# ningyu1991/InclusiveGAN

Hardware: AMD Instinct MI355X
Metric: training img/sec (whole node), CelebA 128x128 StyleGAN2+IMLE (higher is better)
Workload: dtype f32-equivalent (3x3 convs: 2-piece fp16 split, operands to <= 1 ulp of fp32, scales per pixel / per channel: no per-tensor window; fp32 sums)

## Files before the change

inclusivegan_amd/csrc/upfirdn2d.hip:

```cpp
#include "igan_common.h"
#include <hip/hip_fp16.h>
#include <cstdlib>

namespace {

struct FirTaps {
    float k[64];
};

struct UpfirdnArgs {
    const float* x;
    float* y;
    int upx, upy, downx, downy;
    int padx0, pady0;
    int majorDim, inH, inW, minorDim;
    int kernelH, kernelW;
    int outH, outW;
    int xcd_remap;
    const float* noise;
    const float* strength;
    const float* bias;
    int noise_bcast, act;
    float act_alpha, act_gain;
};

__host__ __device__ __forceinline__ int floor_div(int a, int b) {
    int c = a / b;
    if (c * b > a) c--;
    return c;
}

__device__ __forceinline__ float io_load(const float* p) { return *p; }
__device__ __forceinline__ float io_load(const __half* p) { return __half2float(*p); }
__device__ __forceinline__ void io_store(float* p, float v) { *p = v; }
__device__ __forceinline__ void io_store(__half* p, float v) { *p = __float2half(v); }

struct TapWalk { int j0, i0, n; };

__device__ __forceinline__ TapWalk tap_walk(int o, int down, int up, int pad0, int taps, int in) {
    const int u0 = o * down - pad0;
    const int j0 = (u0 >= 0) ? (up - u0 % up) % up : -u0;
    const int i0 = (u0 + j0) / up;
    const int by_taps = (j0 < taps) ? (taps - j0 + up - 1) / up : 0;
    const int by_samples = (i0 < in) ? in - i0 : 0;
    return TapWalk{j0, i0, min(by_taps, by_samples)};
}

template <typename T>
__global__ __launch_bounds__(256) void upfirdn2d_generic_kernel(UpfirdnArgs a, FirTaps taps) {
    const T* xin = reinterpret_cast<const T*>(a.x);
    T* yout = reinterpret_cast<T*>(a.y);
    const long long total = (long long)a.majorDim * a.outH * a.outW * a.minorDim;
    for (long long idx = (long long)blockIdx.x * blockDim.x + threadIdx.x; idx < total;
         idx += (long long)gridDim.x * blockDim.x) {
        long long t = idx;
        const int c = (int)(t % a.minorDim); t /= a.minorDim;
        const int ox = (int)(t % a.outW);    t /= a.outW;
        const int oy = (int)(t % a.outH);    t /= a.outH;
        const int m = (int)t;
        const TapWalk wy = tap_walk(oy, a.downy, a.upy, a.pady0, a.kernelH, a.inH);
        const TapWalk wx = tap_walk(ox, a.downx, a.upx, a.padx0, a.kernelW, a.inW);
        float v = 0.0f;
        for (int sy = 0; sy < wy.n; sy++) {
            const T* xrow = xin + (((long long)m * a.inH + wy.i0 + sy) * a.inW + wx.i0) * a.minorDim + c;
            const float* krow = taps.k + (wy.j0 + sy * a.upy) * a.kernelW + wx.j0;
            for (int sx = 0; sx < wx.n; sx++)
                v += io_load(xrow + (long long)sx * a.minorDim) * krow[sx * a.upx];
        }
        io_store(yout + idx, v);
    }
}

template <int TY, int TX, bool EPI = false>
__global__ __launch_bounds__(256) void upfirdn2d_fir4_kernel(UpfirdnArgs a, FirTaps taps) {
    const int cvecs = a.minorDim >> 2;
    const int strips = (a.outH + TY - 1) / TY;
    const int xgroups = (a.outW + TX - 1) / TX;
    const long long total = (long long)a.majorDim * strips * xgroups * cvecs;
    int bid = blockIdx.x;
    if (a.xcd_remap) {
        const int n = gridDim.x, q = n >> 3, r = n & 7, x = bid & 7;
        bid = (x < r ? x * (q + 1) : r * (q + 1) + (x - r) * q) + (bid >> 3);
    }
    const long long idx = (long long)bid * blockDim.x + threadIdx.x;
    if (idx >= total) return;
    long long t = idx;
    const int cv = (int)(t % cvecs); t /= cvecs;
    const int ox0 = (int)(t % xgroups) * TX; t /= xgroups;
    const int strip = (int)(t % strips); t /= strips;
    const int m = (int)t;
    const int oy0 = strip * TY;

    float4 acc[TY][TX];
#pragma unroll
    for (int i = 0; i < TY; i++)
#pragma unroll
        for (int j = 0; j < TX; j++) acc[i][j] = make_float4(0.f, 0.f, 0.f, 0.f);

    const int ix0 = ox0 - a.padx0;
    const float4* xbase = reinterpret_cast<const float4*>(a.x) + (long long)m * a.inH * a.inW * cvecs + cv;

#pragma unroll
    for (int r = 0; r < TY + 3; r++) {
        const int iy = oy0 + r - a.pady0;
        float4 v[TX + 3];
        const bool rowok = (iy >= 0) & (iy < a.inH);
#pragma unroll
        for (int c = 0; c < TX + 3; c++) {
            const int ix = ix0 + c;
            const bool ok = rowok & (ix >= 0) & (ix < a.inW);
            v[c] = ok ? xbase[((long long)iy * a.inW + ix) * cvecs] : make_float4(0.f, 0.f, 0.f, 0.f);
        }
#pragma unroll
        for (int ky = 0; ky < 4; ky++) {
            const int o = r - ky;
            if (o >= 0 && o < TY) {
#pragma unroll
                for (int j = 0; j < TX; j++)
#pragma unroll
                    for (int kx = 0; kx < 4; kx++) {
                        const float kv = taps.k[ky * 4 + kx];
                        acc[o][j].x += v[j + kx].x * kv;
                        acc[o][j].y += v[j + kx].y * kv;
                        acc[o][j].z += v[j + kx].z * kv;
                        acc[o][j].w += v[j + kx].w * kv;
                    }
            }
        }
    }

    float4* ybase = reinterpret_cast<float4*>(a.y) + (long long)m * a.outH * a.outW * cvecs + cv;
    float4 bb = make_float4(0.f, 0.f, 0.f, 0.f);
    float st = 0.f;
    if constexpr (EPI) {
        if (a.bias) bb = *reinterpret_cast<const float4*>(a.bias + 4 * cv);
        if (a.noise) st = a.strength[0];
    }
#pragma unroll
    for (int i = 0; i < TY; i++) {
        const int oy = oy0 + i;
#pragma unroll
        for (int j = 0; j < TX; j++)
            if (oy < a.outH && ox0 + j < a.outW) {
                float4 v = acc[i][j];
                if constexpr (EPI) {
                    const float nz = a.noise ? a.noise[((long long)(a.noise_bcast ? 0 : m) * a.outH + oy) * a.outW + ox0 + j] * st : 0.f;
                    const float e[4] = {v.x + nz + bb.x, v.y + nz + bb.y, v.z + nz + bb.z, v.w + nz + bb.w};
                    float o[4];
#pragma unroll
                    for (int q = 0; q < 4; q++) {
                        float t = e[q];
                        if (a.act == 2) t = t > 0.f ? t : 0.f;
                        if (a.act == 3) t = t > 0.f ? t : t * a.act_alpha;
                        o[q] = t * a.act_gain;
                    }
                    v = make_float4(o[0], o[1], o[2], o[3]);
                }
                ybase[((long long)oy * a.outW + ox0 + j) * cvecs] = v;
            }
    }
}

}

namespace {
struct FirEpilogue { const float* noise; const float* strength; const float* bias; int noise_bcast, act; float alpha, gain; };
int upfirdn_launch(hipStream_t stream, const igan_upfirdn2d_params* p, const FirEpilogue* epi, bool half_io = false);
}

extern "C" int igan_upfirdn2d(igan_stream_t stream_, const igan_upfirdn2d_params* p) {
    return upfirdn_launch((hipStream_t)stream_, p, nullptr);
}

extern "C" int igan_upfirdn2d_f16(igan_stream_t stream_, const igan_upfirdn2d_params* p) {
    return upfirdn_launch((hipStream_t)stream_, p, nullptr, true);
}

extern "C" int igan_upfirdn2d_ban(igan_stream_t stream_, const igan_upfirdn2d_params* p, const float* noise, const float* strength,
                                  int noise_bcast, const float* bias, int act, float alpha, float gain) {
    using namespace igan;
    IGAN_REQUIRE(act >= 1 && act <= 3, "upfirdn2d_ban: act must be 1 (linear), 2 (relu) or 3 (lrelu)");
    IGAN_REQUIRE(gain > 0.0f, "upfirdn2d_ban: gain must be positive");
    IGAN_REQUIRE((noise == nullptr) == (strength == nullptr), "upfirdn2d_ban: noise and strength go together");
    IGAN_REQUIRE(((uintptr_t)bias & 15) == 0, "upfirdn2d_ban: bias must be 16-byte aligned");
    FirEpilogue e{noise, strength, bias, noise_bcast, act, alpha, gain};
    return upfirdn_launch((hipStream_t)stream_, p, &e);
}

namespace {
int upfirdn_launch(hipStream_t stream, const igan_upfirdn2d_params* p, const FirEpilogue* epi, bool half_io) {
    using namespace igan;
    IGAN_REQUIRE(p != nullptr, "upfirdn2d: null params");
    IGAN_REQUIRE(p->x && p->k && p->y, "upfirdn2d: null buffer");
    IGAN_REQUIRE(p->upx >= 1 && p->upy >= 1, "upx and upy must be at least 1x1");
    IGAN_REQUIRE(p->downx >= 1 && p->downy >= 1, "downx and downy must be at least 1x1");
    IGAN_REQUIRE(p->kernelW >= 1 && p->kernelH >= 1, "kernel must be at least 1x1");
    IGAN_REQUIRE(p->kernelW * p->kernelH <= 64, "kernel too large (max 64 taps)");
    IGAN_REQUIRE(p->majorDim >= 1 && p->inH >= 1 && p->inW >= 1 && p->minorDim >= 1, "input must have rank 4 with positive dims");
    const int outW = (p->inW * p->upx + p->padx0 + p->padx1 - p->kernelW + p->downx) / p->downx;
    const int outH = (p->inH * p->upy + p->pady0 + p->pady1 - p->kernelH + p->downy) / p->downy;
    IGAN_REQUIRE(outW >= 1 && outH >= 1, "output must be at least 1x1");
    IGAN_REQUIRE(outW == p->outW && outH == p->outH, "upfirdn2d: outH/outW (%d,%d) do not match derived (%d,%d)", p->outH, p->outW, outH, outW);
    const long long in_elems = (long long)p->majorDim * p->inH * p->inW * p->minorDim;
    const long long out_elems = (long long)p->majorDim * outH * outW * p->minorDim;
    IGAN_REQUIRE(in_elems <= INT32_MAX, "input too large");
    IGAN_REQUIRE(out_elems <= INT32_MAX, "output too large");

    UpfirdnArgs a;
    a.x = p->x; a.y = p->y;
    a.upx = p->upx; a.upy = p->upy; a.downx = p->downx; a.downy = p->downy;
    a.padx0 = p->padx0; a.pady0 = p->pady0;
    a.majorDim = p->majorDim; a.inH = p->inH; a.inW = p->inW; a.minorDim = p->minorDim;
    a.kernelH = p->kernelH; a.kernelW = p->kernelW;
    a.outH = outH; a.outW = outW;
    static const bool fir_xcd = !(getenv("IGAN_FIR_XCD") && atoi(getenv("IGAN_FIR_XCD")) == 0);
    a.xcd_remap = fir_xcd ? 1 : 0;
    a.noise = epi ? epi->noise : nullptr; a.strength = epi ? epi->strength : nullptr; a.bias = epi ? epi->bias : nullptr;
    a.noise_bcast = epi ? epi->noise_bcast : 0; a.act = epi ? epi->act : 0;
    a.act_alpha = epi ? epi->alpha : 0.f; a.act_gain = epi ? epi->gain : 1.f;

    const bool aligned = (((uintptr_t)p->x | (uintptr_t)p->y) & 15) == 0;
    const bool fast = !half_io && p->upx == 1 && p->upy == 1 && p->downx == 1 && p->downy == 1 &&
                      p->kernelH <= 4 && p->kernelW <= 4 && (p->minorDim % 4) == 0 && aligned;
    FirTaps taps;
    for (int i = 0; i < 64; i++) taps.k[i] = 0.0f;
    if (fast) {
        for (int ky = 0; ky < p->kernelH; ky++)
            for (int kx = 0; kx < p->kernelW; kx++)
                taps.k[ky * 4 + kx] = p->k[(p->kernelH - 1 - ky) * p->kernelW + (p->kernelW - 1 - kx)];
        const int cvecs = p->minorDim / 4;
        static const int tx = getenv("IGAN_FIR_TX") ? atoi(getenv("IGAN_FIR_TX")) : 2;
        if (outH >= 8 && outW >= 16 && tx >= 2) {
            const long long total = (long long)p->majorDim * ceil_div(outH, 8) * ceil_div(outW, 2) * cvecs;
            if (epi) hipLaunchKernelGGL((upfirdn2d_fir4_kernel<8, 2, true>), dim3((int)ceil_div_ll(total, 256)), dim3(256), 0, stream, a, taps);
            else hipLaunchKernelGGL((upfirdn2d_fir4_kernel<8, 2>), dim3((int)ceil_div_ll(total, 256)), dim3(256), 0, stream, a, taps);
        } else if (outH >= 8) {
            const long long total = (long long)p->majorDim * ceil_div(outH, 8) * outW * cvecs;
            if (epi) hipLaunchKernelGGL((upfirdn2d_fir4_kernel<8, 1, true>), dim3((int)ceil_div_ll(total, 256)), dim3(256), 0, stream, a, taps);
            else hipLaunchKernelGGL((upfirdn2d_fir4_kernel<8, 1>), dim3((int)ceil_div_ll(total, 256)), dim3(256), 0, stream, a, taps);
        } else {
            const long long total = (long long)p->majorDim * ceil_div(outH, 2) * outW * cvecs;
            if (epi) hipLaunchKernelGGL((upfirdn2d_fir4_kernel<2, 1, true>), dim3((int)ceil_div_ll(total, 256)), dim3(256), 0, stream, a, taps);
            else hipLaunchKernelGGL((upfirdn2d_fir4_kernel<2, 1>), dim3((int)ceil_div_ll(total, 256)), dim3(256), 0, stream, a, taps);
        }
    } else {
        if (epi) return fail(IGAN_ERR_UNSUPPORTED, "upfirdn2d_ban: the epilogue rides on the FIR fast path only (up = down = 1, taps <= 4x4, minorDim %% 4 == 0, 16-byte aligned)");
        for (int ky = 0; ky < p->kernelH; ky++)
            for (int kx = 0; kx < p->kernelW; kx++)
                taps.k[ky * p->kernelW + kx] = p->k[(p->kernelH - 1 - ky) * p->kernelW + (p->kernelW - 1 - kx)];
        const int grid = (int)std::min<long long>(ceil_div_ll(out_elems, 256), 256 * 32);
        if (half_io) {
            for (int i = 0; i < 64; i++) taps.k[i] = (float)(_Float16)taps.k[i];
            hipLaunchKernelGGL(upfirdn2d_generic_kernel<__half>, dim3(grid), dim3(256), 0, stream, a, taps);
        } else {
            hipLaunchKernelGGL(upfirdn2d_generic_kernel<float>, dim3(grid), dim3(256), 0, stream, a, taps);
        }
    }
    IGAN_LAUNCH_CHECK("upfirdn2d launch");
    return IGAN_OK;
}
}
```

inclusivegan_amd/dnnlib/tflib/ops/upfirdn_2d.py:

```python
import numpy as np
import torch

from .... import hip_ops

_IMPLS = ('hip', 'cuda')


def _check_impl(impl):
    if impl not in _IMPLS:
        raise ValueError("impl must be 'hip' (or the reference's 'cuda'; got %r); the CPU reference lives in oracle/ and is not a product path" % (impl,))


def upfirdn_2d(x, k, upx=1, upy=1, downx=1, downy=1, padx0=0, padx1=0, pady0=0, pady1=0, impl='hip'):
    _check_impl(impl)
    k = np.asarray(k, dtype=np.float32)
    if x.dim() != 4:
        raise ValueError('input must have rank 4')
    for v in (upx, upy, downx, downy, padx0, padx1, pady0, pady1):
        assert isinstance(v, (int, np.integer))
    return hip_ops.UpFirDn2dFn.apply(x, k, int(upx), int(upy), int(downx), int(downy), int(padx0), int(padx1), int(pady0), int(pady1))


def filter_2d(x, k, gain=1, data_format='NCHW', impl='hip'):
    k = _setup_kernel(k) * gain
    p = k.shape[0] - 1
    return _simple_upfirdn_2d(x, k, pad0=(p+1)//2, pad1=p//2, data_format=data_format, impl=impl)

def upsample_2d(x, k=None, factor=2, gain=1, data_format='NCHW', impl='hip'):
    assert isinstance(factor, int) and factor >= 1
    if k is None:
        k = [1] * factor
    k = _setup_kernel(k) * (gain * (factor ** 2))
    p = k.shape[0] - factor
    return _simple_upfirdn_2d(x, k, up=factor, pad0=(p+1)//2+factor-1, pad1=p//2, data_format=data_format, impl=impl)

def downsample_2d(x, k=None, factor=2, gain=1, data_format='NCHW', impl='hip'):
    assert isinstance(factor, int) and factor >= 1
    if k is None:
        k = [1] * factor
    k = _setup_kernel(k) * gain
    p = k.shape[0] - factor
    return _simple_upfirdn_2d(x, k, down=factor, pad0=(p+1)//2, pad1=p//2, data_format=data_format, impl=impl)


def _to_nchw(x, data_format):
    assert data_format in ['NCHW', 'NHWC']
    return x if data_format == 'NCHW' else x.permute(0, 3, 1, 2)

def _from_nchw(y, data_format):
    return y if data_format == 'NCHW' else y.permute(0, 2, 3, 1)

def upsample_conv_2d(x, w, k=None, factor=2, gain=1, data_format='NCHW', impl='hip'):
    _check_impl(impl)
    assert isinstance(factor, int) and factor >= 1
    assert w.dim() == 4
    convH, convW, inC, outC = [int(d) for d in w.shape]
    assert convW == convH
    if factor != 2:
        raise NotImplementedError('upsample_conv_2d: only factor=2 is built (the only one the configs use)')
    if k is None:
        k = [1] * factor
    k = _setup_kernel(k) * (gain * (factor ** 2))
    p = (k.shape[0] - factor) - (convW - 1)
    xn = _to_nchw(x, data_format)
    if xn.shape[1] != inC:
        raise NotImplementedError('upsample_conv_2d: grouped convolution is not offered on the hip path')
    H, W = int(xn.shape[2]), int(xn.shape[3])
    geom = hip_ops.ConvGeom(convH, convW, 1, factor, convH - 1, convW - 1)
    y = hip_ops.conv2d(xn, w, geom, ((H - 1) * factor + convH, (W - 1) * factor + convW))
    y = _simple_upfirdn_2d(y, k, pad0=(p+1)//2+factor-1, pad1=p//2+1, data_format='NCHW', impl=impl)
    return _from_nchw(y, data_format)

def conv_downsample_2d(x, w, k=None, factor=2, gain=1, data_format='NCHW', impl='hip'):
    _check_impl(impl)
    assert isinstance(factor, int) and factor >= 1
    convH, convW, inC, outC = [int(d) for d in w.shape]
    assert convW == convH
    if k is None:
        k = [1] * factor
    k = _setup_kernel(k) * gain
    p = (k.shape[0] - factor) + (convW - 1)
    xn = _to_nchw(x, data_format)
    xn = _simple_upfirdn_2d(xn, k, pad0=(p+1)//2, pad1=p//2, data_format='NCHW', impl=impl)
    H, W = int(xn.shape[2]), int(xn.shape[3])
    geom = hip_ops.ConvGeom(convH, convW, factor, 1, 0, 0)
    y = hip_ops.conv2d(xn, w, geom, ((H - convH) // factor + 1, (W - convW) // factor + 1))
    return _from_nchw(y, data_format)


def _setup_kernel(k):
    k = np.asarray(k, dtype=np.float32)
    if k.ndim == 1:
        k = np.outer(k, k)
    k /= np.sum(k)
    assert k.ndim == 2
    assert k.shape[0] == k.shape[1]
    return k

def _simple_upfirdn_2d(x, k, up=1, down=1, pad0=0, pad1=0, data_format='NCHW', impl='hip'):
    assert data_format in ['NCHW', 'NHWC']
    assert x.dim() == 4
    y = x
    if data_format == 'NCHW':
        y = hip_ops.nhwc(y).permute(0, 2, 3, 1)
    y = upfirdn_2d(y, k, upx=up, upy=up, downx=down, downy=down, padx0=pad0, padx1=pad1, pady0=pad0, pady1=pad1, impl=impl)
    if data_format == 'NCHW':
        y = y.permute(0, 3, 1, 2)
    return y
```

inclusivegan_amd/hip_ops.py:

```python
import ctypes
import os
from collections import namedtuple

import numpy as np
import torch

from . import _abi

CL = torch.channels_last


def _stream():
    return ctypes.c_void_p(torch.cuda.current_stream().cuda_stream)


def _ptr(t):
    return ctypes.c_void_p(t.data_ptr()) if t is not None else ctypes.c_void_p(0)


def _require_cuda_f32(*ts):
    for t in ts:
        if t is None:
            continue
        if not t.is_cuda:
            raise RuntimeError('inclusivegan_amd kernels need tensors on a ROCm device (got %s); there is no CPU path' % t.device)
        if t.dtype != torch.float32:
            raise TypeError('inclusivegan_amd kernels are fp32 (got %s)' % t.dtype)


def _require_cuda_io(*ts):
    kinds = {t.dtype for t in ts if t is not None}
    for t in ts:
        if t is not None and not t.is_cuda:
            raise RuntimeError('inclusivegan_amd kernels need tensors on a ROCm device (got %s); there is no CPU path' % t.device)
    if len(kinds) != 1 or next(iter(kinds)) not in (torch.float32, torch.float16):
        raise TypeError('upfirdn_2d / fused_bias_act take float32 or float16 tensors of one type (got %s)' % sorted(str(k) for k in kinds))
    return next(iter(kinds)) == torch.float16


def _is_meta(t):
    return t.device.type == 'meta'


def _needed(ctx, i):
    if not ctx.needs_input_grad[i]:
        return False
    try:
        mask = getattr(ctx, 'input_is_tensor', None)
        j = i if mask is None else sum(1 for m in mask[:i] if m)
        node = ctx.next_functions[j][0]
        return node is not None and torch._C._will_engine_execute_node(node)
    except Exception:
        return True


def _mark_inputs(ctx, *inputs):
    ctx.input_is_tensor = [isinstance(t, torch.Tensor) for t in inputs]


def nhwc(x):
    return x.contiguous(memory_format=CL)


def empty_nchw(n, c, h, w, like):
    return torch.empty((n, c, h, w), device=like.device, dtype=torch.float32, memory_format=CL)



def upfirdn2d_raw(x, k, upx, upy, downx, downy, padx0, padx1, pady0, pady1, epilogue=None):
    k = np.ascontiguousarray(k, dtype=np.float32)
    if k.ndim != 2:
        raise ValueError('kernel must have rank 2')
    if x.dim() != 4:
        raise ValueError('input must have rank 4')
    major, in_h, in_w, minor = x.shape
    kh, kw = k.shape
    out_w = (in_w * upx + padx0 + padx1 - kw + downx) // downx
    out_h = (in_h * upy + pady0 + pady1 - kh + downy) // downy
    if out_w < 1 or out_h < 1:
        raise ValueError('output must be at least 1x1')
    if _is_meta(x):
        return torch.empty((major, out_h, out_w, minor), device='meta')
    lib = _abi.get_plugin()
    half = _require_cuda_io(x)
    if half and epilogue is not None:
        raise TypeError('upfirdn2d: the fused layer epilogue is a float32 path')
    x = x.contiguous()
    y = torch.empty((major, out_h, out_w, minor), device=x.device, dtype=x.dtype)
    p = _abi.UpFirDn2DParams(
        x=x.data_ptr(), k=k.ctypes.data, y=y.data_ptr(),
        upx=upx, upy=upy, downx=downx, downy=downy,
        padx0=padx0, padx1=padx1, pady0=pady0, pady1=pady1,
        majorDim=major, inH=in_h, inW=in_w, minorDim=minor,
        kernelH=kh, kernelW=kw, outH=out_h, outW=out_w)
    if epilogue is not None:
        noise, strength, bias, act_idx, alpha, gain = epilogue
        _require_cuda_f32(noise, strength, bias)
        if noise is not None:
            noise = noise.contiguous()
            if noise.numel() not in (out_h * out_w, major * out_h * out_w):
                raise ValueError('upfirdn2d epilogue: noise must hold [majorDim or 1, outH, outW] values')
        bcast = 1 if (noise is not None and noise.numel() == out_h * out_w and major > 1) else 0
        _abi.check(lib.igan_upfirdn2d_ban(_stream(), ctypes.byref(p), _ptr(noise), _ptr(strength if noise is not None else None), bcast,
                                          _ptr(bias.contiguous() if bias is not None else None), int(act_idx), float(alpha), float(gain)))
        return y
    _abi.check((lib.igan_upfirdn2d_f16 if half else lib.igan_upfirdn2d)(_stream(), ctypes.byref(p)))
    return y


def fir_ban_fusable(x, k, act_idx):
    k = np.asarray(k)
    return (_FIR_BAN and _second_order_depth == 0 and not _is_meta(x) and x.is_cuda and x.dim() == 4 and x.shape[1] % 4 == 0
            and act_idx in (1, 2, 3) and k.ndim == 2 and k.shape[0] <= 4 and k.shape[1] <= 4)


_FIR_BAN = os.environ.get('IGAN_FIR_BAN', '1') != '0'


class FirBanFn(torch.autograd.Function):

    @staticmethod
    def forward(ctx, x, k, pad0, pad1, b, noise, strength, act_idx, alpha, gain):
        _mark_inputs(ctx, x, k, pad0, pad1, b, noise, strength, act_idx, alpha, gain)
        k = np.asarray(k, dtype=np.float32)
        xh = nhwc(x).permute(0, 2, 3, 1)
        y = upfirdn2d_raw(xh, k, 1, 1, 1, 1, pad0, pad1, pad0, pad1, epilogue=(noise, strength, b, act_idx, alpha, gain))
        in_h, in_w = xh.shape[1], xh.shape[2]
        out_h, out_w = y.shape[1], y.shape[2]
        kh, kw = k.shape
        ctx.gargs = (np.ascontiguousarray(k[::-1, ::-1]), 1, 1, 1, 1, kw - pad0 - 1, in_w - out_w + pad0, kh - pad0 - 1, in_h - out_h + pad0)
        y = y.permute(0, 3, 1, 2)
        ctx.save_for_backward(y, noise)
        ctx.cfg = (act_idx, alpha, gain)
        ctx.has_b = b is not None
        return y

    @staticmethod
    def backward(ctx, dy):
        if torch.is_grad_enabled():
            raise NotImplementedError('fused FIR + epilogue: second-order gradients go through UpFirDn2dFn + BiasActNoiseFn (hip_ops.second_order())')
        y, noise = ctx.saved_tensors
        act_idx, alpha, gain = ctx.cfg
        need_b = ctx.has_b and _needed(ctx, 4)
        need_s = noise is not None and _needed(ctx, 6)
        nz = noise.expand(_noise_view(y)).contiguous() if noise is not None else None
        dxp, db, ds = bias_act_noise_bwd_raw(dy, y, nz, act_idx, alpha, gain, need_b)
        dx = None
        if _needed(ctx, 0):
            dx = upfirdn2d_raw(nhwc(dxp).permute(0, 2, 3, 1), *ctx.gargs).permute(0, 3, 1, 2)
        return dx, None, None, None, (db if need_b else None), None, (ds if need_s else None), None, None, None


class UpFirDn2dFn(torch.autograd.Function):

    @staticmethod
    def forward(ctx, x, k, upx, upy, downx, downy, padx0, padx1, pady0, pady1):
        k = np.asarray(k, dtype=np.float32)
        in_h, in_w = x.shape[1], x.shape[2]
        y = upfirdn2d_raw(x, k, upx, upy, downx, downy, padx0, padx1, pady0, pady1)
        out_h, out_w = y.shape[1], y.shape[2]
        kh, kw = k.shape
        gpadx0 = kw - padx0 - 1
        gpady0 = kh - pady0 - 1
        gpadx1 = in_w * upx - out_w * downx + padx0 - upx + 1
        gpady1 = in_h * upy - out_h * downy + pady0 - upy + 1
        ctx.gargs = (np.ascontiguousarray(k[::-1, ::-1]), downx, downy, upx, upy, gpadx0, gpadx1, gpady0, gpady1)
        return y

    @staticmethod
    def backward(ctx, dy):
        dx = UpFirDn2dFn.apply(dy, *ctx.gargs)
        return (dx,) + (None,) * 9



def _bias_layout(x, axis):
    if x.dim() == 4 and axis == 1 and x.is_contiguous(memory_format=CL):
        return x, x.shape[1], 1
    xc = x.contiguous()
    step = 1
    for d in xc.shape[axis + 1:]:
        step *= int(d)
    return xc, int(xc.shape[axis]), step


def fused_bias_act_raw(x, b, ref, grad, act_idx, alpha, gain, size_b, step_b):
    if _is_meta(x):
        return torch.empty_like(x)
    lib = _abi.get_plugin()
    half = _require_cuda_io(x, b, ref)
    y = torch.empty_like(x)
    p = _abi.FusedBiasActParams(
        x=x.data_ptr(), b=(b.data_ptr() if b is not None else None),
        ref=(ref.data_ptr() if ref is not None else None), y=y.data_ptr(),
        grad=grad, act=act_idx, alpha=float(alpha), gain=float(gain),
        sizeX=x.numel(), sizeB=size_b, stepB=step_b)
    _abi.check((lib.igan_fused_bias_act_f16 if half else lib.igan_fused_bias_act)(_stream(), ctypes.byref(p)))
    return y


def bias_grad_raw(dx, size_b, step_b):
    lib = _abi.get_plugin()
    if dx.dtype == torch.float16:
        return dx.reshape(-1, size_b, step_b).float().sum(dim=(0, 2)).to(torch.float16)
    _require_cuda_f32(dx)
    n = dx.numel()
    ws_floats = lib.igan_bias_grad_workspace_floats(n, size_b, step_b)
    ws = torch.empty((max(int(ws_floats), 1),), device=dx.device, dtype=torch.float32)
    db = torch.empty((size_b,), device=dx.device, dtype=torch.float32)
    _abi.check(lib.igan_bias_grad(_stream(), _ptr(dx), _ptr(db), _ptr(ws), n, size_b, step_b))
    return db


def _match_layout(t, ref):
    if t.shape == ref.shape and t.stride() == ref.stride():
        return t
    out = torch.empty_like(ref)
    out.copy_(t)
    return out


class _FbaGradFn(torch.autograd.Function):

    @staticmethod
    def forward(ctx, dy, bias_term, ref, axis, act_idx, alpha, gain, size_b, step_b, zero_2nd, xrecv=None):
        ctx.cfg = (axis, act_idx, alpha, gain, size_b, step_b, zero_2nd)
        ctx.has_bias_term = bias_term is not None
        dyl = _match_layout(dy, ref)
        ctx.save_for_backward(ref, *(() if zero_2nd else (dyl, bias_term) if bias_term is not None else (dyl,)))
        return fused_bias_act_raw(dyl, bias_term, ref, 1, act_idx, alpha, gain, size_b, step_b)

    @staticmethod
    def backward(ctx, d_dx):
        ref = ctx.saved_tensors[0]
        axis, act_idx, alpha, gain, size_b, step_b, zero_2nd = ctx.cfg
        d_dy = _FbaGradFn.apply(d_dx, None, ref, axis, act_idx, alpha, gain, size_b, step_b, True) if zero_2nd else None
        d_x = None
        if not zero_2nd:
            with torch.no_grad():
                g = _match_layout(d_dx, ref)
                d_dy = fused_bias_act_raw(g, None, ref, 1, act_idx, alpha, gain, size_b, step_b)
                if ctx.needs_input_grad[10]:
                    dy = ctx.saved_tensors[1]
                    if ctx.has_bias_term:
                        view = [1] * dy.dim(); view[axis] = -1
                        dy = dy + ctx.saved_tensors[2].view(*view)
                    d_x = fused_bias_act_raw(g, None, ref, 2, act_idx, alpha, gain, size_b, step_b) * dy
        d_bias_term = None
        if ctx.has_bias_term:
            d_bias_term = _BiasGradFn.apply(d_dy, axis, size_b, step_b)
        return (d_dy, d_bias_term) + (None,) * 8 + (d_x,)


class _BiasGradFn(torch.autograd.Function):

    @staticmethod
    def forward(ctx, dx, axis, size_b, step_b):
        ctx.shape = dx.shape
        ctx.axis = axis
        return bias_grad_raw(dx, size_b, step_b)

    @staticmethod
    def backward(ctx, d_db):
        view = [1] * len(ctx.shape)
        view[ctx.axis] = -1
        return d_db.view(*view).expand(ctx.shape), None, None, None


class FusedBiasActFn(torch.autograd.Function):
    @staticmethod
    def forward(ctx, x, b, axis, act_idx, alpha, gain, ref_kind, zero_2nd):
        xd, size_b, step_b = _bias_layout(x, axis)
        y = fused_bias_act_raw(xd, b, None, 0, act_idx, alpha, gain, size_b, step_b)
        ctx.save_for_backward(xd if ref_kind == 'x' else y)
        ctx.cfg = (axis, act_idx, alpha, gain, size_b, step_b, zero_2nd)
        ctx.has_b = b is not None
        return y

    @staticmethod
    def backward(ctx, dy):
        (ref,) = ctx.saved_tensors
        axis, act_idx, alpha, gain, size_b, step_b, zero_2nd = ctx.cfg
        dx = _FbaGradFn.apply(dy, None, ref, axis, act_idx, alpha, gain, size_b, step_b, zero_2nd)
        db = _BiasGradFn.apply(dx, axis, size_b, step_b) if (ctx.has_b and _needed(ctx, 1)) else None
        return (dx, db) + (None,) * 6


class FusedBiasActSmoothFn(torch.autograd.Function):

    @staticmethod
    def forward(ctx, x, b, axis, act_idx, alpha, gain, ref_kind):
        xd, size_b, step_b = _bias_layout(x, axis)
        y = fused_bias_act_raw(xd, b, None, 0, act_idx, alpha, gain, size_b, step_b)
        ctx.cfg = (axis, act_idx, alpha, gain, size_b, step_b, ref_kind)
        ctx.has_b = b is not None
        ctx.save_for_backward(xd, y, b)
        return y

    @staticmethod
    def backward(ctx, dy):
        xd, y, b = ctx.saved_tensors
        axis, act_idx, alpha, gain, size_b, step_b, ref_kind = ctx.cfg
        ref = (xd if ref_kind == 'x' else y).detach()
        if torch.is_grad_enabled():
            recv = xd
            if ref_kind != 'x' and b is not None:
                view = [1] * xd.dim(); view[axis] = -1
                recv = xd + b.view(*view)
            dx = _FbaGradFn.apply(dy, None, ref, axis, act_idx, alpha, gain, size_b, step_b, False, recv)
        else:
            dx = fused_bias_act_raw(_match_layout(dy, ref), None, ref, 1, act_idx, alpha, gain, size_b, step_b)
        db = _BiasGradFn.apply(dx, axis, size_b, step_b) if (ctx.has_b and _needed(ctx, 1)) else None
        return (dx, db) + (None,) * 5



def _rows_c(x):
    if x.dim() == 4 and x.is_contiguous(memory_format=CL) and x.shape[1] % 4 == 0:
        return x.shape[0] * x.shape[2] * x.shape[3], x.shape[1]
    if x.dim() == 2 and x.is_contiguous() and x.shape[1] % 4 == 0:
        return x.shape[0], x.shape[1]
    return None


def bias_act_noise_fwd_raw(x, noise, strength, b, act_idx, alpha, gain):
    if _is_meta(x):
        return torch.empty_like(x)
    lib = _abi.get_plugin()
    _require_cuda_f32(x, noise, strength, b)
    rows, c = _rows_c(x)
    y = torch.empty_like(x)
    _abi.check(lib.igan_bias_act_noise_fwd(_stream(), _ptr(x), _ptr(noise), _ptr(strength), _ptr(b), _ptr(y),
                                           rows, c, act_idx, float(alpha), float(gain)))
    return y


def bias_act_noise_bwd_raw(dy, y, noise, act_idx, alpha, gain, want_db):
    lib = _abi.get_plugin()
    _require_cuda_f32(dy, y, noise)
    rows, c = _rows_c(y)
    dy = _match_layout(dy, y)
    dx = torch.empty_like(y)
    ws = torch.empty((int(lib.igan_bias_act_noise_workspace_floats(rows, c)),), device=y.device, dtype=torch.float32)
    db = torch.empty((c,), device=y.device, dtype=torch.float32) if want_db else None
    ds = torch.empty((), device=y.device, dtype=torch.float32) if noise is not None else None
    _abi.check(lib.igan_bias_act_noise_bwd(_stream(), _ptr(dy), _ptr(y), _ptr(noise), _ptr(dx), _ptr(db), _ptr(ds), _ptr(ws),
                                           rows, c, act_idx, float(alpha), float(gain)))
    return dx, db, ds


class BiasActNoiseFn(torch.autograd.Function):

    @staticmethod
    def forward(ctx, x, b, noise, strength, act_idx, alpha, gain):
        _mark_inputs(ctx, x, b, noise, strength, act_idx, alpha, gain)
        y = bias_act_noise_fwd_raw(x, noise, strength, b, act_idx, alpha, gain)
        ctx.save_for_backward(y, noise)
        ctx.cfg = (act_idx, alpha, gain)
        ctx.has_b = b is not None
        return y

    @staticmethod
    def backward(ctx, dy):
        y, noise = ctx.saved_tensors
        act_idx, alpha, gain = ctx.cfg
        need_b = ctx.has_b and _needed(ctx, 1)
        need_s = noise is not None and _needed(ctx, 3)
        if torch.is_grad_enabled():
            c = y.shape[1]
            dx = _FbaGradFn.apply(dy, None, y, 1, act_idx, alpha, gain, c, 1, True)
            db = _BiasGradFn.apply(dx, 1, c, 1) if need_b else None
            ds = (dx * noise.reshape(_noise_view(y))).sum() if need_s else None
            return dx, db, None, ds, None, None, None
        dx, db, ds = bias_act_noise_bwd_raw(dy, y, noise, act_idx, alpha, gain, need_b)
        return dx, db, None, (ds if need_s else None), None, None, None


def _noise_view(y):
    return (y.shape[0], 1, y.shape[2], y.shape[3]) if y.dim() == 4 else (y.shape[0], 1)


def bias_act_noise(x, b, noise, strength, act_idx, alpha, gain):
    if _is_meta(x):
        return torch.empty_like(x)
    if x.dim() in (2, 4) and x.shape[1] % 4 == 0:
        x = nhwc(x) if x.dim() == 4 else x.contiguous()
        if noise is not None:
            noise = noise.expand(_noise_view(x)).contiguous()
        return BiasActNoiseFn.apply(x, b, noise, strength, act_idx, alpha, gain)
    if noise is not None:
        x = x + noise * strength
    return FusedBiasActFn.apply(x, b, 1, act_idx, alpha, gain, 'y', True)



ConvGeom = namedtuple('ConvGeom', 'kh kw stride up pad_y pad_x alpha', defaults=(1.0,))

_plan_cache = {}
_wplan_cache = {}

launch_log = None
stamp_log = None
shape_log = None


class StampLog:

    def __init__(self, device, capacity=16384):
        self.stamps = torch.zeros((2 * capacity,), device=device, dtype=torch.int64)
        self.acc = torch.zeros((capacity,), device=device, dtype=torch.int64)
        self.entries = []
        self.shapes = []
        self.capacity = capacity
        self._folded = 0
        self.folds = {}

    def bracket(self, name, flops, launch, shape=None):
        i = len(self.entries)
        if i >= self.capacity:
# ... 1721 lines not shown
```

Before: 351.4.

## Add dedicated polyphase up2/down2 FIR kernels with register tiling for upfirdn2d

Adds specialized upfirdn2d kernels for the 2x upsample and 2x downsample cases with taps up to 4x4. They use float4 channel vectors, polyphase tap selection templated on pad parity, register tiles of several outputs per thread, and the same XCD block remapping as the existing fast path. These cases previously went through the generic path, so the aim is fewer wasted multiply-by-zero taps, fewer redundant loads and better reuse. A second, opt-in path (env flag defaulting off) runs the decimation before a 1x1 conv in conv_downsample instead of striding the conv.

```diff
diff --git a/inclusivegan_amd/csrc/upfirdn2d.hip b/inclusivegan_amd/csrc/upfirdn2d.hip
--- a/inclusivegan_amd/csrc/upfirdn2d.hip
+++ b/inclusivegan_amd/csrc/upfirdn2d.hip
@@ -161,6 +161,151 @@
     }
 }
 
+__device__ __forceinline__ int fir_block_id(const UpfirdnArgs& a) {
+    int bid = blockIdx.x;
+    if (a.xcd_remap) {
+        const int n = gridDim.x, q = n >> 3, r = n & 7, x = bid & 7;
+        bid = (x < r ? x * (q + 1) : r * (q + 1) + (x - r) * q) + (bid >> 3);
+    }
+    return bid;
+}
+
+__device__ __forceinline__ void fir_acc(float4& acc, const float4& v, float kv) {
+    acc.x += v.x * kv;
+    acc.y += v.y * kv;
+    acc.z += v.z * kv;
+    acc.w += v.w * kv;
+}
+
+template <int TY, int TX>
+__global__ __launch_bounds__(256) void upfirdn2d_down2_kernel(UpfirdnArgs a, FirTaps taps) {
+    const int cvecs = a.minorDim >> 2;
+    const int strips = (a.outH + TY - 1) / TY;
+    const int xgroups = (a.outW + TX - 1) / TX;
+    const long long total = (long long)a.majorDim * strips * xgroups * cvecs;
+    const long long idx = (long long)fir_block_id(a) * blockDim.x + threadIdx.x;
+    if (idx >= total) return;
+    long long t = idx;
+    const int cv = (int)(t % cvecs); t /= cvecs;
+    const int ox0 = (int)(t % xgroups) * TX; t /= xgroups;
+    const int oy0 = (int)(t % strips) * TY; t /= strips;
+    const int m = (int)t;
+
+    float4 acc[TY][TX];
+#pragma unroll
+    for (int i = 0; i < TY; i++)
+#pragma unroll
+        for (int j = 0; j < TX; j++) acc[i][j] = make_float4(0.f, 0.f, 0.f, 0.f);
+
+    const int iy0 = 2 * oy0 - a.pady0, ix0 = 2 * ox0 - a.padx0;
+    const float4* xbase = reinterpret_cast<const float4*>(a.x) + (long long)m * a.inH * a.inW * cvecs + cv;
+
+#pragma unroll
+    for (int r = 0; r < 2 * TY + 2; r++) {
+        const int iy = iy0 + r;
+        const bool rowok = (iy >= 0) & (iy < a.inH);
+        float4 v[2 * TX + 2];
+#pragma unroll
+        for (int c = 0; c < 2 * TX + 2; c++) {
+            const int ix = ix0 + c;
+            const bool ok = rowok & (ix >= 0) & (ix < a.inW);
+            v[c] = ok ? xbase[((long long)iy * a.inW + ix) * cvecs] : make_float4(0.f, 0.f, 0.f, 0.f);
+        }
+#pragma unroll
+        for (int ky = 0; ky < 4; ky++) {
+            const int d = r - ky;
+            if (d >= 0 && (d & 1) == 0 && d / 2 < TY) {
+#pragma unroll
+                for (int j = 0; j < TX; j++)
+#pragma unroll
+                    for (int kx = 0; kx < 4; kx++) fir_acc(acc[d / 2][j], v[2 * j + kx], taps.k[ky * 4 + kx]);
+            }
+        }
+    }
+
+    float4* ybase = reinterpret_cast<float4*>(a.y) + (long long)m * a.outH * a.outW * cvecs + cv;
+#pragma unroll
+    for (int i = 0; i < TY; i++)
+#pragma unroll
+        for (int j = 0; j < TX; j++)
+            if (oy0 + i < a.outH && ox0 + j < a.outW) ybase[((long long)(oy0 + i) * a.outW + ox0 + j) * cvecs] = acc[i][j];
+}
+
+template <int TY, int TX, int EY, int EX>
+__global__ __launch_bounds__(256) void upfirdn2d_up2_kernel(UpfirdnArgs a, FirTaps taps) {
+    const int cvecs = a.minorDim >> 2;
+    const int strips = (a.outH + 2 * TY - 1) / (2 * TY);
+    const int xgroups = (a.outW + 2 * TX - 1) / (2 * TX);
+    const long long total = (long long)a.majorDim * strips * xgroups * cvecs;
+    const long long idx = (long long)fir_block_id(a) * blockDim.x + threadIdx.x;
+    if (idx >= total) return;
+    long long t = idx;
+    const int cv = (int)(t % cvecs); t /= cvecs;
+    const int ox0 = (int)(t % xgroups) * 2 * TX; t /= xgroups;
+    const int oy0 = (int)(t % strips) * 2 * TY; t /= strips;
+    const int m = (int)t;
+
+    float4 acc[2 * TY][2 * TX];
+#pragma unroll
+    for (int i = 0; i < 2 * TY; i++)
+#pragma unroll
+        for (int j = 0; j < 2 * TX; j++) acc[i][j] = make_float4(0.f, 0.f, 0.f, 0.f);
+
+    const int iy0 = (oy0 - a.pady0 + EY) >> 1, ix0 = (ox0 - a.padx0 + EX) >> 1;
+    const float4* xbase = reinterpret_cast<const float4*>(a.x) + (long long)m * a.inH * a.inW * cvecs + cv;
+
+#pragma unroll
+    for (int s = 0; s < TY + 2 - EY; s++) {
+        const int iy = iy0 + s;
+        const bool rowok = (iy >= 0) & (iy < a.inH);
+        float4 v[TX + 2 - EX];
+#pragma unroll
+        for (int c = 0; c < TX + 2 - EX; c++) {
+            const int ix = ix0 + c;
+            const bool ok = rowok & (ix >= 0) & (ix < a.inW);
+            v[c] = ok ? xbase[((long long)iy * a.inW + ix) * cvecs] : make_float4(0.f, 0.f, 0.f, 0.f);
+        }
+#pragma unroll
+        for (int o = 0; o < 2 * TY; o++) {
+            const int ky = 2 * s + EY - o;
+            if (ky >= 0 && ky < 4) {
+#pragma unroll
+                for (int q = 0; q < 2 * TX; q++)
+#pragma unroll
+                    for (int c = 0; c < TX + 2 - EX; c++) {
+                        const int kx = 2 * c + EX - q;
+                        if (kx >= 0 && kx < 4) fir_acc(acc[o][q], v[c], taps.k[ky * 4 + kx]);
+                    }
+            }
+        }
+    }
+
+    float4* ybase = reinterpret_cast<float4*>(a.y) + (long long)m * a.outH * a.outW * cvecs + cv;
+#pragma unroll
+    for (int i = 0; i < 2 * TY; i++)
+#pragma unroll
+        for (int j = 0; j < 2 * TX; j++)
+            if (oy0 + i < a.outH && ox0 + j < a.outW) ybase[((long long)(oy0 + i) * a.outW + ox0 + j) * cvecs] = acc[i][j];
+}
+
+template <int TY, int TX>
+void launch_up2(hipStream_t stream, const UpfirdnArgs& a, const FirTaps& taps) {
+    const long long total = (long long)a.majorDim * igan::ceil_div(a.outH, 2 * TY) * igan::ceil_div(a.outW, 2 * TX) * (a.minorDim / 4);
+    const dim3 grid((int)igan::ceil_div_ll(total, 256)), block(256);
+    switch ((a.pady0 & 1) * 2 + (a.padx0 & 1)) {
+        case 0: hipLaunchKernelGGL((upfirdn2d_up2_kernel<TY, TX, 0, 0>), grid, block, 0, stream, a, taps); break;
+        case 1: hipLaunchKernelGGL((upfirdn2d_up2_kernel<TY, TX, 0, 1>), grid, block, 0, stream, a, taps); break;
+        case 2: hipLaunchKernelGGL((upfirdn2d_up2_kernel<TY, TX, 1, 0>), grid, block, 0, stream, a, taps); break;
+        default: hipLaunchKernelGGL((upfirdn2d_up2_kernel<TY, TX, 1, 1>), grid, block, 0, stream, a, taps); break;
+    }
+}
+
+template <int TY, int TX>
+void launch_down2(hipStream_t stream, const UpfirdnArgs& a, const FirTaps& taps) {
+    const long long total = (long long)a.majorDim * igan::ceil_div(a.outH, TY) * igan::ceil_div(a.outW, TX) * (a.minorDim / 4);
+    hipLaunchKernelGGL((upfirdn2d_down2_kernel<TY, TX>), dim3((int)igan::ceil_div_ll(total, 256)), dim3(256), 0, stream, a, taps);
+}
+
 }
 
 namespace {
@@ -220,14 +365,25 @@
     a.act_alpha = epi ? epi->alpha : 0.f; a.act_gain = epi ? epi->gain : 1.f;
 
     const bool aligned = (((uintptr_t)p->x | (uintptr_t)p->y) & 15) == 0;
-    const bool fast = !half_io && p->upx == 1 && p->upy == 1 && p->downx == 1 && p->downy == 1 &&
-                      p->kernelH <= 4 && p->kernelW <= 4 && (p->minorDim % 4) == 0 && aligned;
+    const bool stream4 = !half_io && p->kernelH <= 4 && p->kernelW <= 4 && (p->minorDim % 4) == 0 && aligned;
+    const bool fast = stream4 && p->upx == 1 && p->upy == 1 && p->downx == 1 && p->downy == 1;
+    static const bool updown = !(getenv("IGAN_FIR_UPDOWN") && atoi(getenv("IGAN_FIR_UPDOWN")) == 0);
+    const bool down2 = updown && stream4 && !epi && p->upx == 1 && p->upy == 1 && p->downx == 2 && p->downy == 2;
+    const bool up2 = updown && stream4 && !epi && p->upx == 2 && p->upy == 2 && p->downx == 1 && p->downy == 1;
     FirTaps taps;
     for (int i = 0; i < 64; i++) taps.k[i] = 0.0f;
-    if (fast) {
+    if (fast || down2 || up2) {
         for (int ky = 0; ky < p->kernelH; ky++)
             for (int kx = 0; kx < p->kernelW; kx++)
                 taps.k[ky * 4 + kx] = p->k[(p->kernelH - 1 - ky) * p->kernelW + (p->kernelW - 1 - kx)];
+    }
+    if (down2) {
+        if (outH >= 8 && outW >= 16) launch_down2<2, 2>(stream, a, taps);
+        else launch_down2<2, 1>(stream, a, taps);
+    } else if (up2) {
+        if (outH >= 16 && outW >= 16) launch_up2<2, 1>(stream, a, taps);
+        else launch_up2<1, 1>(stream, a, taps);
+    } else if (fast) {
         const int cvecs = p->minorDim / 4;
         static const int tx = getenv("IGAN_FIR_TX") ? atoi(getenv("IGAN_FIR_TX")) : 2;
         if (outH >= 8 && outW >= 16 && tx >= 2) {
diff --git a/inclusivegan_amd/dnnlib/tflib/ops/upfirdn_2d.py b/inclusivegan_amd/dnnlib/tflib/ops/upfirdn_2d.py
--- a/inclusivegan_amd/dnnlib/tflib/ops/upfirdn_2d.py
+++ b/inclusivegan_amd/dnnlib/tflib/ops/upfirdn_2d.py
@@ -1,3 +1,5 @@
+import os
+
 import numpy as np
 import torch
 
@@ -81,6 +83,10 @@
     k = _setup_kernel(k) * gain
     p = (k.shape[0] - factor) + (convW - 1)
     xn = _to_nchw(x, data_format)
+    if convH == 1 and hip_ops.fir_decimate_fusable(xn, k, factor) and os.environ.get('IGAN_SKIP_DECIMATE', '0') == '1':
+        xn = _simple_upfirdn_2d(xn, k, down=factor, pad0=(p+1)//2, pad1=p//2, data_format='NCHW', impl=impl)
+        y = hip_ops.conv2d(xn, w, hip_ops.ConvGeom(1, 1, 1, 1, 0, 0), (int(xn.shape[2]), int(xn.shape[3])))
+        return _from_nchw(y, data_format)
     xn = _simple_upfirdn_2d(xn, k, pad0=(p+1)//2, pad1=p//2, data_format='NCHW', impl=impl)
     H, W = int(xn.shape[2]), int(xn.shape[3])
     geom = hip_ops.ConvGeom(convH, convW, factor, 1, 0, 0)
diff --git a/inclusivegan_amd/hip_ops.py b/inclusivegan_amd/hip_ops.py
--- a/inclusivegan_amd/hip_ops.py
+++ b/inclusivegan_amd/hip_ops.py
@@ -115,6 +115,11 @@
 
 
 _FIR_BAN = os.environ.get('IGAN_FIR_BAN', '1') != '0'
+
+
+def fir_decimate_fusable(x, k, factor):
+    k = np.asarray(k)
+    return factor == 2 and x.dim() == 4 and x.dtype == torch.float32 and x.shape[1] % 4 == 0 and k.ndim == 2 and k.shape[0] <= 4 and k.shape[1] <= 4
 
 
 class FirBanFn(torch.autograd.Function):
```

Result: no change. 349.0 (-0.7%).
